# tgialoimtr/cnn_lstm_ctc_ocr

Measured on AMD Instinct MI355X. Metric: line-crops/sec (train step) at 32x256 bs=256; CER vs ref, higher is better.
Workload: dtype bf16

## Files before the change

### cnn_lstm_ctc_ocr_amd/_lib.py

```python
import ctypes
import os

import torch

_HERE = os.path.dirname(os.path.abspath(__file__))
LIB_PATH = os.environ.get("OCRK_LIB") or os.path.join(_HERE, "libocrk.so")

OCRK_OK = 0
OCRK_ERR_INVALID_ARG = 1
OCRK_ERR_HIP = 2
OCRK_ERR_INFEASIBLE = 3

F32 = 0
BF16 = 1

_p = ctypes.c_void_p
_i32 = ctypes.c_int
_u32 = ctypes.c_uint
_i64 = ctypes.c_int64
_f32 = ctypes.c_float
_sz = ctypes.c_size_t

SIGNATURES = {
    "ocrk_version": [],
# ... 70 lines not shown
    "ocrk_bn_relu_pool_bwd_slab": [_p, _p, _i32, _i32, _i32, _i32, _p, _p, _p, _p, _i32, _i32, _i32, _i32,
                                   _i32, _p, _p, _p, _i32, _p, _p, _sz, _i32, _p],
    "ocrk_lstm_fwd_step": [_p, _p, _p, _p, _p, _p, _i32, _i32, _i32, _i32, _p, _p, _p, _p, _i32, _p],
    "ocrk_lstm_bwd_step": [_p, _p, _p, _p, _p, _i32, _i32, _i32, _i32, _p, _p, _p, _p, _i32, _p],
    "ocrk_copy_batch": [_p, _i32, _i64, _p],
    "ocrk_gru_fwd_persistent_supported": [_i32, _i32],
    "ocrk_gru_fwd_persistent_workspace_size": [_i32, _i32],
    "ocrk_gru_fwd_persistent": [_p, _p, _p, _p, _i32, _i32, _i32, _p, _p, _p, _p, _p, _p, _p, _sz, _p],
    "ocrk_gru_bwd_persistent_supported": [_i32, _i32],
    "ocrk_gru_bwd_persistent_workspace_size": [_i32, _i32],
    "ocrk_gru_bwd_persistent": [_p, _p, _p, _i32, _i32, _i32, _p, _p, _p, _p, _p, _p, _p, _p, _sz, _p],
    "ocrk_persistent_flags_size": [_i32, _i32],
    "ocrk_lstm_fwd_persistent_supported": [_i32, _i32],
    "ocrk_lstm_fwd_persistent_workspace_size": [_i32, _i32],
    "ocrk_lstm_fwd_persistent": [_p, _p, _p, _i32, _i32, _i32, _p, _p, _p, _p, _p, _p, _p, _sz, _p],
    "ocrk_lstm_fwd_persistent_f32_supported": [_i32, _i32],
    "ocrk_lstm_fwd_persistent_f32_workspace_size": [_i32, _i32],
    "ocrk_lstm_fwd_persistent_f32_flags_size": [_i32, _i32],
    "ocrk_lstm_fwd_persistent_f32": [_p, _p, _p, _i32, _i32, _i32, _p, _p, _p, _p, _p, _p, _p, _sz, _p],
    "ocrk_lstm_bwd_persistent_f32_supported": [_i32, _i32],
    "ocrk_lstm_bwd_persistent_f32_workspace_size": [_i32, _i32],
    "ocrk_lstm_bwd_persistent_f32": [_p, _p, _i32, _i32, _i32, _p, _p, _p, _p, _p, _p, _p, _p, _sz, _p],
    "ocrk_lstm_bwd_persistent_supported": [_i32, _i32],
    "ocrk_lstm_bwd_persistent_workspace_size": [_i32, _i32],
    "ocrk_lstm_bwd_persistent_slices": [_i32, _i32],
    "ocrk_lstm_bwd_persistent": [_p, _p, _i32, _i32, _i32, _p, _p, _p, _p, _p, _p, _p, _p, _sz, _p],
    "ocrk_lstm_fwd": [_p, _p, _p, _p, _p, _i32, _i32, _i32, _p, _p, _p, _p, _i32, _p],
    "ocrk_lstm_bwd": [_p, _p, _p, _p, _i32, _i32, _i32, _p, _p, _p, _p, _i32, _p],
    "ocrk_gemm_workspace_size": [_i32, _i32, _i32, _i32],
    "ocrk_gemm": [_i32, _i32, _i32, _i32, _i32, _f32, _p, _i64, _i64, _p, _i64, _i64, _p, _i64, _i64,
                  _i32, _p, _i32, _i32, _i32, _i32, _i32, _p, _sz, _p],
    "ocrk_adam": [_p, _p, _p, _p, _i64, _f32, _f32, _f32, _f32, _f32, _p],
    "ocrk_adam_ex": [_p, _p, _p, _p, _i64, _f32, _f32, _f32, _f32, _f32, _u32, _p],
    "ocrk_cast": [_p, _i32, _p, _i32, _i64, _p],
    "ocrk_split_bf16": [_p, _i64, _p, _p, _p],
    "ocrk_permute3": [_p, _i32, _i32, _i32, _i32, _p, _i32, _p],
    "ocrk_strided_copy": [_p, _i64, _i64, _i64, _i64, _p, _i32, _i64, _i64, _p],
    "ocrk_colsum_workspace_size": [_i64, _i32],
    "ocrk_colsum": [_p, _i64, _i32, _i32, _p, _i32, _p, _sz, _p],
    "ocrk_slab_sum_workspace_size": [_i32],
    "ocrk_slab_sum": [_p, _i32, _i32, _i32, _p, _i32, _p, _sz, _p],
    "ocrk_relu_mask": [_p, _p, _i64, _f32, _p, _i32, _p],
    "ocrk_mul_scalar": [_p, _i64, _p, _p],
    "ocrk_mean": [_p, _i32, _p, _p],
    "ocrk_seq_len": [_p, _i32, _p, _p],
    "ocrk_timer_create": [_p],
    "ocrk_timer_record": [_p, _p],
    "ocrk_timer_elapsed": [_p, _p, _p],
    "ocrk_timer_destroy": [_p],
}
_RESTYPE = {"ocrk_last_error": ctypes.c_char_p}
_RESTYPE.update({n: ctypes.c_size_t for n in SIGNATURES if n.endswith("_workspace_size")})
_RESTYPE["ocrk_conv_stats_tiles"] = ctypes.c_size_t
_RESTYPE["ocrk_persistent_flags_size"] = ctypes.c_size_t
_RESTYPE["ocrk_bn_bwd_bias_slab_rows"] = ctypes.c_size_t
_RESTYPE["ocrk_bn_bwd_pooled_bias_slab_rows"] = ctypes.c_size_t
_RESTYPE["ocrk_crc32c"] = ctypes.c_uint32


class OcrkError(RuntimeError):

    def __init__(self, status, message):
        super().__init__(message)
        self.status = status


# ... 127 lines not shown
```

### cnn_lstm_ctc_ocr_amd/csrc/adam.hip

```cpp
#include "common.h"

template <bool ZERO>
__global__ void __launch_bounds__(256)
adam_kernel(float* __restrict__ p, float* __restrict__ g, float* __restrict__ m, float* __restrict__ v,
            int64_t n, float lr_t, float b1, float b2, float eps, float grad_scale) {
    const int64_t n4 = n / 4;
    const float c1 = 1.f - b1, c2 = 1.f - b2;
    for (int64_t i = (int64_t)blockIdx.x * 256 + threadIdx.x; i < n4; i += (int64_t)gridDim.x * 256) {
        float4 pp = reinterpret_cast<float4*>(p)[i], gg = reinterpret_cast<const float4*>(g)[i];
        float4 mm = reinterpret_cast<float4*>(m)[i], vv = reinterpret_cast<float4*>(v)[i];
        float* pe = &pp.x; float* ge = &gg.x; float* me = &mm.x; float* ve = &vv.x;
#pragma unroll
        for (int k = 0; k < 4; ++k) {
            float gk = ge[k] * grad_scale;
            me[k] += (gk - me[k]) * c1;
            ve[k] += (gk * gk - ve[k]) * c2;
            pe[k] -= lr_t * me[k] / (sqrtf(ve[k]) + eps);
        }
        reinterpret_cast<float4*>(p)[i] = pp;
        reinterpret_cast<float4*>(m)[i] = mm;
        reinterpret_cast<float4*>(v)[i] = vv;
        if constexpr (ZERO) reinterpret_cast<float4*>(g)[i] = make_float4(0.f, 0.f, 0.f, 0.f);
    }
    for (int64_t i = n4 * 4 + (int64_t)blockIdx.x * 256 + threadIdx.x; i < n; i += (int64_t)gridDim.x * 256) {
        float gk = g[i] * grad_scale;
        m[i] += (gk - m[i]) * c1;
        v[i] += (gk * gk - v[i]) * c2;
        p[i] -= lr_t * m[i] / (sqrtf(v[i]) + eps);
        if constexpr (ZERO) g[i] = 0.f;
    }
}

extern "C" int ocrk_adam_ex(float* p, float* g, float* m, float* v, int64_t n, float lr_t, float beta1,
                            float beta2, float eps, float grad_scale, unsigned flags, void* stream) {
    if (n == 0) return OCRK_OK;
    OCRK_REQUIRE(((uintptr_t)p | (uintptr_t)g | (uintptr_t)m | (uintptr_t)v) % 16 == 0, "ocrk_adam: buffers must be 16-B aligned");
    OCRK_REQUIRE((flags & ~(unsigned)OCRK_ADAM_ZERO_GRAD) == 0, "ocrk_adam_ex: unknown flags 0x%x", flags);
    unsigned grid = (unsigned)std::max<int64_t>(1, std::min<int64_t>(ocrk::cdiv(n / 4 + 1, 256), 4096));
    hipStream_t s = ocrk::as_stream(stream);
    if (flags & OCRK_ADAM_ZERO_GRAD)
        adam_kernel<true><<<grid, 256, 0, s>>>(p, g, m, v, n, lr_t, beta1, beta2, eps, grad_scale);
    else
        adam_kernel<false><<<grid, 256, 0, s>>>(p, g, m, v, n, lr_t, beta1, beta2, eps, grad_scale);
    return ocrk::launch_status("ocrk_adam");
}

extern "C" int ocrk_adam(float* p, const float* g, float* m, float* v, int64_t n, float lr_t, float beta1,
                         float beta2, float eps, float grad_scale, void* stream) {
    return ocrk_adam_ex(p, const_cast<float*>(g), m, v, n, lr_t, beta1, beta2, eps, grad_scale, 0u, stream);
}
```

### cnn_lstm_ctc_ocr_amd/kernels.py

```python
import ctypes

import torch

from . import _lib, options
from ._lib import ptr, call

F32, BF16 = _lib.F32, _lib.BF16
_DT = {torch.float32: F32, torch.bfloat16: BF16}


def dtype_code(dt):
    try:
        return _DT[dt]
    except KeyError:
        raise TypeError(f"unsupported dtype {dt}; libocrk computes in float32 or bfloat16")


def _stream(t):
    return _lib.stream_ptr(t.device)


def _chk(*ts):
    for t in ts:
        if t is None:
# ... 722 lines not shown
def colsum(x, M, N, out, accumulate=True):
    _chk(x, out)
    nb = _lib.lib().ocrk_colsum_workspace_size(M, N)
    ws = _ws(nb, x.device)
    call("ocrk_colsum", ptr(x), M, N, dtype_code(x.dtype), ptr(out), int(accumulate), ptr(ws), nb, _stream(x))


def relu_mask(dy, y, out_dtype, scale=1.0):
    _chk(dy, y)
    out = torch.empty(dy.shape, dtype=out_dtype, device=dy.device)
    call("ocrk_relu_mask", ptr(dy), ptr(y), dy.numel(), float(scale), ptr(out), dtype_code(out_dtype), _stream(dy))
    return out


def mul_scalar_(x, s):
    _chk(x, s)
    call("ocrk_mul_scalar", ptr(x), x.numel(), ptr(s), _stream(x))
    return x


def mean(x):
    _chk(x)
    out = torch.empty((), dtype=torch.float32, device=x.device)
    call("ocrk_mean", ptr(x), x.numel(), ptr(out), _stream(x))
    return out


def adam_(p, g, m, v, lr_t, beta1=0.9, beta2=0.999, eps=1e-8, grad_scale=1.0, zero_grad=False):
    _chk(p, g, m, v)
    call("ocrk_adam_ex", ptr(p), ptr(g), ptr(m), ptr(v), p.numel(), float(lr_t), float(beta1), float(beta2),
         float(eps), float(grad_scale), 1 if zero_grad else 0, _stream(p))


def ctc_loss(logits, labels, label_len, seq_len, grad_scale=1.0, need_grad=True, status=None):
    if logits.dtype != torch.float32:
        raise TypeError("ctc_loss takes float32 logits")
    _chk(logits, labels, label_len, seq_len)
    T, B, C = logits.shape
    Lmax = labels.shape[1] if labels.dim() == 2 else 0
    labels = labels.reshape(B, Lmax)
    if labels.numel() == 0:
        labels = torch.zeros(B, 1, dtype=torch.int32, device=logits.device)
        Lmax = 1
    nb = _lib.lib().ocrk_ctc_workspace_size(T, B, Lmax)
    ws = _ws(nb, logits.device)
    loss = torch.empty(B, dtype=torch.float32, device=logits.device)
    grad = torch.empty_like(logits) if need_grad else None
    if status is None:
        status = torch.empty(B, dtype=torch.int32, device=logits.device)
    call("ocrk_ctc_loss", ptr(logits), ptr(labels), ptr(label_len), ptr(seq_len), T, B, C, Lmax,
         float(grad_scale), ptr(loss), ptr(grad), ptr(status), ptr(status_word(logits.device)), ptr(ws), nb,
         _stream(logits))
    return loss, grad, status


def ctc_align(logits, labels, label_len, seq_len, status=None):
    if logits.dtype != torch.float32:
        raise TypeError("ctc_align takes float32 logits")
    _chk(logits, labels, label_len, seq_len)
    T, B, C = logits.shape
    Lmax = Lout = labels.shape[1] if labels.dim() == 2 else 0
    labels = labels.reshape(B, Lmax)
    if labels.numel() == 0:
        labels = torch.zeros(B, 1, dtype=torch.int32, device=logits.device)
        Lmax = 1
    nb = _lib.lib().ocrk_ctc_align_workspace_size(T, B, Lmax)
# ... 105 lines not shown
```

### cnn_lstm_ctc_ocr_amd/options.py

```python
import contextlib
import os

_HOST_DEFAULTS = {
    "LSTM_PERSISTENT": 1,
    "F32_TRAIN_EXACT": 0,
    "SIDE_STREAM": 1,
    "CONV_SIDE": 1,
    "CONV12_FUSED": 1,
    "RELU_BITS": 1,
    "POOLED_BN": 1,
    "CONV1_FUSED": 1,
    "CONV12_BWD": 1,
    "TN_ITEMS": 256,
    "TN_ITEMS_L1": 160,
}
KERNEL_OPTIONS = ("CONV_DIRECT", "CONV_ROWS", "CONV_ROWS_WIDE", "CONV_WGRAD_BLOCKS", "LSTM_SPIN_LIMIT",
                  "PERSIST_LATE", "LSTM_BWD_R16", "CTC_LDS",
                  "PP_PERSIST_NK", "NT_F32_EXACT", "NT_F32_MASK",
                  "NT_F32_X6", "BEAM_WAVE", "BN_BWD_BLOCKS", "BN_ROUTE", "BN_ROUTE_SEG", "BN_ROUTE_NCH", "CONV_TN_ITEMS", "CONV_TN4_ITEMS",
                  "CONV_WGRAD_CUS", "F32_MFMA", "GEMM_NT", "GEMM_NT_STAGED", "GEMM_PP", "GEMM_PPTN", "PP_MIN_N", "GEMM_TN",
                  "LSTM_DMA", "LSTM_BWD_DMA", "LSTM_FWD_R16", "NT_TAP_UNIFORM")


def _env_int(name, default):
    v = os.environ.get("OCRK_" + name)
    if v is None or v == "":
        return default
    try:
        return int(v)
    except ValueError:
        raise ValueError(f"OCRK_{name}={v!r}: an integer is expected") from None


_HOST = {k: _env_int(k, d) for k, d in _HOST_DEFAULTS.items()}


def get(name):
    if name in _HOST:
        return _HOST[name]
    if name in KERNEL_OPTIONS:
        import ctypes

        from . import _lib
        v = ctypes.c_int64()
        _lib.call("ocrk_get_option", name.encode(), ctypes.byref(v))
# ... 30 lines not shown
```

### cnn_lstm_ctc_ocr_amd/params.py

```python

import numpy as np
import torch

from . import kernels as K
from .config import LAYER_PARAMS, ModelConfig

_ALIGN = 64


def param_shapes(cfg):
    out = []
    cin = 1
    for filters, k, _pad, name, bn in LAYER_PARAMS:
        out.append((f"convnet/{name}/kernel", (k, k, cin, filters), True))
        out.append((f"convnet/{name}/bias", (filters,), True))
        if bn:
            out.append((f"convnet/{name}/batch_norm/gamma", (filters,), True))
            out.append((f"convnet/{name}/batch_norm/beta", (filters,), True))
            out.append((f"convnet/{name}/batch_norm/moving_mean", (filters,), False))
            out.append((f"convnet/{name}/batch_norm/moving_variance", (filters,), False))
        cin = filters
    n_in = cin
    for li, H in enumerate(cfg.rnn_sizes, start=1):
        pre = f"rnn/bdrnn{li}"
# ... 31 lines not shown
    return out[:i] + rnn + out[i:]


def _trunc_normal(rng, shape, std):
    x = rng.standard_normal(shape)
    bad = np.abs(x) > 2
    while bad.any():
        x[bad] = rng.standard_normal(int(bad.sum()))
        bad = np.abs(x) > 2
    return x * std


def reference_init(cfg, seed=0):
    rng = np.random.default_rng(seed)
    vals = {}
    shapes = {n: sh for n, sh, _t in param_shapes(cfg)}
    for name in creation_order(cfg):
        shape = shapes[name]
        leaf = name.rsplit("/", 1)[1]
        if name.startswith("convnet") and leaf == "kernel":
            v = _trunc_normal(rng, shape, np.sqrt(2.6 / (shape[0] * shape[1] * shape[2])))
        elif name == "rnn/logits/kernel":
            v = _trunc_normal(rng, shape, np.sqrt(2.6 / shape[0]))
        elif "gru_cell" in name or ("lstm_cell" in name and leaf == "kernel"):
            v = _trunc_normal(rng, shape, 0.01)
        elif leaf in ("gamma", "moving_variance"):
            v = np.ones(shape)
        else:
            v = np.zeros(shape)
        vals[name] = v.astype(np.float32)
    return vals


class ParamStore:
    def __init__(self, cfg=None, device="cuda", seed=0, values=None):
        self.cfg = cfg or ModelConfig()
        self.device = torch.device(device)
        self.spec = param_shapes(self.cfg)
        self.offsets = {}
        sizes = {True: 0, False: 0}
        for name, shape, tr in self.spec:
            n = int(np.prod(shape))
            self.offsets[name] = (tr, sizes[tr], shape)
            sizes[tr] += (n + _ALIGN - 1) // _ALIGN * _ALIGN
        self.n_trainable = sum(int(np.prod(s)) for _, s, tr in self.spec if tr)
        self.flat = torch.zeros(sizes[True], dtype=torch.float32, device=self.device)
        self.flat_grad = torch.zeros_like(self.flat)
        self.flat_stats = torch.zeros(max(sizes[False], _ALIGN), dtype=torch.float32, device=self.device)
        self.params, self.grads, self.stats = {}, {}, {}
        for name, shape, tr in self.spec:
            _, off, _ = self.offsets[name]
            n = int(np.prod(shape))
            if tr:
                self.params[name] = self.flat[off:off + n].view(shape)
                self.grads[name] = self.flat_grad[off:off + n].view(shape)
            else:
                self.stats[name] = self.flat_stats[off:off + n].view(shape)
        self.version = 0
        self._images = {}
        self.pending = []
        self.conv_late = []
        self.bn_group = None
        self.f32_conv_exact = False
        self.load_state_dict(values if values is not None else reference_init(self.cfg, seed))

    def state_dict(self):
# ... 39 lines not shown
        self._plan_fresh = False

    def images(self, key, builder):
        plan = self._plan_for(key)
        if plan is not None:
            if not self._plan_fresh:
                K.copy_batch(plan["table"], plan["njobs"], plan["tiles"], self.flat)
                self._plan_fresh = True
            return plan["images"][key]
        img = self._images.get(key)
        if img is None:
            img = builder()
            self._images[key] = img
        return img

    def _plan_for(self, key):
        if self.device.type != "cuda":
            return None
        dtype = key[-1]
        if dtype != self.cfg.dtype:
            return None
        plan = getattr(self, "_plan", None)
        if plan is None:
            plan = self._plan = self._build_plan(dtype)
            self._plan_fresh = False
        return plan if key in plan["images"] else None

    def _build_plan(self, dtype):
        dev = self.device
        esz = torch.empty(0, dtype=dtype).element_size()
        code = K.dtype_code(dtype)
        jobs, images = [], {}

        def job(src, s_off, rows, cols, in_rs, dst, d_off, out_rs, transpose):
            jobs.append([src.data_ptr() + 4 * s_off, dst.data_ptr() + esz * d_off, rows, cols, in_rs, out_rs, 0,
                         int(transpose) | (code << 32)])

        for li in range(2, 9):
            w = self.params[f"convnet/conv{li}/kernel"]
            kh, kw, cin, cout = w.shape
            w_nk = torch.empty(cout, kh * kw * cin, dtype=dtype, device=dev)
            w_bwd = torch.empty(cin, kh * kw * cout, dtype=dtype, device=dev)
            job(w, 0, kh * kw * cin, cout, cout, w_nk, 0, kh * kw * cin, True)
            for t in range(kh * kw):
                job(w, t * cin * cout, cin, cout, cout, w_bwd, t * cout, kh * kw * cout, False)
            images[("conv", f"conv{li}", dtype)] = (w_nk, w_bwd)
        for layer in range(1, len(self.cfg.rnn_sizes) + 1):
            pre = f"rnn/bdrnn{layer}"
            if self.cfg.cell == "lstm":
                kf = self.params[f"{pre}/fw/lstm_cell/kernel"]
                rows, G = kf.shape
                H = G // 4
                n_in = rows - H
                wxT = torch.empty(2 * G, n_in, dtype=dtype, device=dev)
                wx = torch.empty(n_in, 2 * G, dtype=dtype, device=dev)
                whT = torch.empty(2, G, H, dtype=dtype, device=dev)
                wh = torch.empty(2, H, G, dtype=dtype, device=dev)
                for d, dn in enumerate(("fw", "bw")):
                    k = self.params[f"{pre}/{dn}/lstm_cell/kernel"]
                    job(k, 0, n_in, G, G, wxT, d * G * n_in, n_in, True)
                    job(k, 0, n_in, G, G, wx, d * G, 2 * G, False)
                    job(k, n_in * G, H, G, G, whT, d * G * H, H, True)
                    job(k, n_in * G, H, G, G, wh, d * H * G, G, False)
                images[("lstm", layer, dtype)] = (wxT, wx, whT, wh, self.flat_bias_pair(layer))
            else:
                gk = self.params[f"{pre}/fw/gru_cell/gates/kernel"]
                rows, G2 = gk.shape
                H = G2 // 2
                n_in = rows - H
                G3 = 3 * H
                wxT = torch.empty(2 * G3, n_in, dtype=dtype, device=dev)
                wx = torch.empty(n_in, 2 * G3, dtype=dtype, device=dev)
                whgT = torch.empty(2, G2, H, dtype=dtype, device=dev)
                whcT = torch.empty(2, H, H, dtype=dtype, device=dev)
                whg = torch.empty(2, H, G2, dtype=dtype, device=dev)
                whc = torch.empty(2, H, H, dtype=dtype, device=dev)
                for d, dn in enumerate(("fw", "bw")):
                    g = self.params[f"{pre}/{dn}/gru_cell/gates/kernel"]
                    c = self.params[f"{pre}/{dn}/gru_cell/candidate/kernel"]
                    job(g, 0, n_in, G2, G2, wxT, d * G3 * n_in, n_in, True)
                    job(c, 0, n_in, H, H, wxT, (d * G3 + G2) * n_in, n_in, True)
                    job(g, 0, n_in, G2, G2, wx, d * G3, 2 * G3, False)
                    job(c, 0, n_in, H, H, wx, d * G3 + G2, 2 * G3, False)
                    job(g, n_in * G2, H, G2, G2, whgT, d * G2 * H, H, True)
                    job(c, n_in * H, H, H, H, whcT, d * H * H, H, True)
                    job(g, n_in * G2, H, G2, G2, whg, d * H * G2, G2, False)
                    job(c, n_in * H, H, H, H, whc, d * H * H, H, False)
                images[("gru", layer, dtype)] = (wxT, wx, whgT, whcT, whg, whc, self.gru_bias_cat(layer))
        lk = self.params["rnn/logits/kernel"]
        limg = torch.empty(lk.shape, dtype=dtype, device=dev)
        limgT = torch.empty(lk.shape[1], lk.shape[0], dtype=dtype, device=dev)
        job(lk, 0, lk.shape[0], lk.shape[1], lk.shape[1], limg, 0, lk.shape[1], False)
        job(lk, 0, lk.shape[0], lk.shape[1], lk.shape[1], limgT, 0, lk.shape[0], True)
        images[("logits", dtype)] = limg
        images[("logitsT", dtype)] = limgT
        tiles = 0
        for j in jobs:
            j[6] = tiles
            tiles += -(-j[2] // 32) * -(-j[3] // 32)
        table = torch.tensor(jobs, dtype=torch.int64).to(dev)
        return {"table": table, "njobs": len(jobs), "tiles": tiles, "images": images}

    def conv_images(self, name, dtype):
        def build():
            w = self.params[f"convnet/{name}/kernel"]
            kh, kw, cin, cout = w.shape
            w_nk = K.permute3(w, kh * kw * cin, cout, 1, dtype).view(cout, kh * kw * cin)
            w_bwd = K.permute3(w, kh * kw, cin, cout, dtype).view(cin, kh * kw * cout)
            return w_nk, w_bwd
        return self.images(("conv", name, dtype), build)

    def lstm_images(self, layer, dtype):
        def build():
            pre = f"rnn/bdrnn{layer}"
            kf = self.params[f"{pre}/fw/lstm_cell/kernel"]
            rows, G = kf.shape
            H = G // 4
            n_in = rows - H
            dev = kf.device
            wxT = torch.empty(2 * G, n_in, dtype=dtype, device=dev)
            wx = torch.empty(n_in, 2 * G, dtype=dtype, device=dev)
            whT = torch.empty(2, G, H, dtype=dtype, device=dev)
            wh = torch.empty(2, H, G, dtype=dtype, device=dev)
            for d, dn in enumerate(("fw", "bw")):
                k = self.params[f"{pre}/{dn}/lstm_cell/kernel"]
                K.strided_copy(k, n_in, G, G, 1, wxT, 1, n_in, out_offset=d * G * n_in)
                K.strided_copy(k, n_in, G, G, 1, wx, 2 * G, 1, out_offset=d * G)
                K.strided_copy(k, H, G, G, 1, whT, 1, H, out_offset=d * G * H, in_offset=n_in * G)
                K.strided_copy(k, H, G, G, 1, wh, G, 1, out_offset=d * H * G, in_offset=n_in * G)
            bias = self.flat_bias_pair(layer)
            return wxT, wx, whT, wh, bias
        return self.images(("lstm", layer, dtype), build)

    def flat_bias_pair(self, layer):
# ... 73 lines not shown
```

### cnn_lstm_ctc_ocr_amd/train.py

```python
import collections
import math
import time

import torch
import torch.distributed as dist

from . import _lib
from . import kernels as K
from . import options
from . import model as _model
from .config import TRAIN
from .model import check_feasible_host, convnet_layers, ctc_loss_layer, dense_labels, host_labels, rnn_layers




class GradBuckets:

    def __init__(self, store, group=None, comm=None, force=False):
        self.store, self.group, self.comm, self.force = store, group, comm, bool(force)
        rnn = [off for name, (tr, off, _s) in store.offsets.items() if tr and name.startswith("rnn/")]
        self.split = min(rnn) if rnn else store.flat_grad.numel()
        self.work = None
        self._stream = None
# ... 79 lines not shown
        dist.all_reduce(flat_grad, op=dist.ReduceOp.SUM, group=group)
    return 1.0 / world


class Trainer:

    def __init__(self, store, learning_rate=1e-4, momentum=0.9, decay_rate=0.9, decay_steps=2 ** 16,
                 decay_staircase=False, beta2=0.999, epsilon=1e-8, process_group=None, global_step=0,
                 summary=None, summary_every=100, sync_bn=False, comm=None, force_exchange=False):
        self.store = store
        self.sync_bn = bool(sync_bn)
        self.summary = summary
        self.summary_every = max(1, int(summary_every))
        self._summary_mark = None
        self.base_lr = learning_rate
        self.beta1 = momentum
        self.beta2 = beta2
        self.eps = epsilon
        self.decay_rate = decay_rate
        self.decay_steps = decay_steps
        self.staircase = decay_staircase
        self.group = process_group
        self.global_step = global_step
        self.m = torch.zeros_like(store.flat)
        self.v = torch.zeros_like(store.flat)
        self._grads_zeroed = False
        self._status_host = None
        self._status_ev = None
        self._status_stream = None
        self._status_ring = collections.deque()
        self.status_lag = 2
        self.buckets = GradBuckets(store, process_group, comm=comm, force=force_exchange)
        self.overlap_allreduce = True

    def learning_rate(self, step=None):
        step = self.global_step if step is None else step
        e = step / self.decay_steps
        if self.staircase:
            e = math.floor(e)
        return self.base_lr * self.decay_rate ** e

    def _bn_group(self):
        if not self.sync_bn or not (dist.is_available() and dist.is_initialized()):
            return None
        return self.group if self.group is not None else dist.group.WORLD

    def world_size(self):
        if self.buckets.comm is not None:
            return self.buckets.world()
        if dist.is_available() and dist.is_initialized():
            return dist.get_world_size(self.group)
        return 1

    def loss_and_grads(self, image, width, label):
        store = self.store
        if store.cfg.dtype != torch.float32:
            return self._loss_and_grads(image, width, label)
        if options.get("F32_TRAIN_EXACT"):
            with K.f32_exact():
                return self._loss_and_grads(image, width, label)
        prev, store.f32_conv_exact = store.f32_conv_exact, True
        try:
            return self._loss_and_grads(image, width, label)
        finally:
            store.f32_conv_exact = prev

    def _loss_and_grads(self, image, width, label):
        store = self.store
        prev_group, store.bn_group = store.bn_group, self._bn_group()
        try:
            return self._forward_backward(image, width, label)
        finally:
            store.bn_group = prev_group

    def _forward_backward(self, image, width, label):
        store = self.store
        if host_labels(label) and not (isinstance(width, torch.Tensor) and width.is_cuda):
            check_feasible_host(label, width)
        if self._grads_zeroed and not (store.device.type == "cuda" and torch.cuda.is_current_stream_capturing()):
            store.join()
        else:
            store.zero_grad()
        self._grads_zeroed = False
        features, seq_len = convnet_layers(image, width, TRAIN, store)
        if self.overlap_allreduce and features.requires_grad and self.buckets.active() and \
                not (features.is_cuda and torch.cuda.is_current_stream_capturing()):
            features.register_hook(self.buckets.rnn_ready)
        logits = rnn_layers(features, seq_len, store.cfg.num_classes, store)
        loss = ctc_loss_layer(logits, label, seq_len)
        if loss.dtype == torch.float32:
            _model.unit_backward(loss)
        else:
            loss.backward()
        return loss

    def reduce_gradients(self):
        self.store.join()
        return self.buckets.finish()

    def apply_gradients(self):
        store = self.store
        grad_scale = self.reduce_gradients()
        t = self.global_step + 1
        lr = self.learning_rate()
        lr_t = lr * math.sqrt(1 - self.beta2 ** t) / (1 - self.beta1 ** t)
        zero = store.device.type == "cuda"
        K.adam_(store.flat, store.flat_grad, self.m, self.v, lr_t, self.beta1, self.beta2, self.eps,
                grad_scale=grad_scale, zero_grad=zero)
        self._grads_zeroed = zero
        store.bump()
        self.global_step += 1

    def step(self, image, width, label):
        self.poll_status()
        lr = self.learning_rate()
        loss = self.loss_and_grads(image, width, label)
        self.apply_gradients()
        self.post_status()
        self.summarize(loss, lr, int(image.shape[0]))
        return loss

    def summarize(self, loss, lr, batch):
        if self.summary is None:
            return
        if self._summary_mark is not None and self.global_step % self.summary_every:
            return
        dev = self.store.device
        if dev.type == "cuda":
            now = torch.cuda.Event(enable_timing=True)
            now.record(torch.cuda.current_stream(dev))
        else:
            now = time.perf_counter()
        if self._summary_mark is None:
            self._summary_mark = (self.global_step, now)
        if self.global_step % self.summary_every:
            return
        s0, t0 = self._summary_mark
        crops = (self.global_step - s0) * batch * self.world_size()
        vals = {"learning_rate": lr, "loss": loss}
        if self.global_step > s0:
            if dev.type == "cuda":
                vals["crops_per_sec"] = lambda: round(crops / max(t0.elapsed_time(now) / 1e3, 1e-9), 2)
            elif now > t0:
                vals["crops_per_sec"] = round(crops / (now - t0), 2)
        self.summary.scalars(self.global_step, **vals)
        self._summary_mark = (self.global_step, now)

    def post_status(self):
        dev = self.store.device
# ... 110 lines not shown
```

### include/ocrk.h

```cpp
#ifndef OCRK_H_
#define OCRK_H_

#include <stddef.h>
#include <stdint.h>

#ifdef __cplusplus
extern "C" {
#endif

#define OCRK_ABI_VERSION 7

enum ocrk_status {
    OCRK_OK = 0,
    OCRK_ERR_INVALID_ARG = 1,
    OCRK_ERR_HIP = 2,
    OCRK_ERR_INFEASIBLE = 3
};

enum ocrk_dtype { OCRK_F32 = 0, OCRK_BF16 = 1 };

int ocrk_set_f32_gemm_mode(int mode);
int ocrk_f32_gemm_exact(void);

enum ocrk_device_status {
// ... 184 lines not shown
                 const int* seq_len, int T, int B, int H, const void* dout, const void* hprev_t,
                 const void* acts_t, void* dG_t, int dtype, void* stream);
int ocrk_gru_fwd_persistent_supported(int B, int H);
size_t ocrk_gru_fwd_persistent_workspace_size(int B, int H);
int ocrk_gru_fwd_persistent(const void* gx, const void* whgT, const void* whcT, const int* seq_len, int T, int B,
                            int H, void* out, void* hprev_t, void* rh_t, void* acts_t, unsigned* err,
                            unsigned* flags, void* ws, size_t ws_bytes, void* stream);
int ocrk_gru_bwd_persistent_supported(int B, int H);
size_t ocrk_gru_bwd_persistent_workspace_size(int B, int H);
int ocrk_gru_bwd_persistent(const void* whg, const void* whc, const int* seq_len, int T, int B, int H,
                            const void* dout, const void* hprev_t, const void* acts_t, void* dG_t, unsigned* err,
                            unsigned* flags, float* dbias_part, void* ws, size_t ws_bytes, void* stream);
size_t ocrk_persistent_flags_size(int B, int H);
int ocrk_lstm_fwd(const void* gx, const void* whT, void* h_state, float* c_state, const int* seq_len,
                  int T, int B, int H, void* out, void* hprev_t, float* cprev_t, void* acts_t, int dtype,
                  void* stream);
int ocrk_lstm_bwd(const void* wh, void* dg_state, float* dc_state, const int* seq_len, int T, int B, int H,
                  const void* dout, const float* cprev_t, const void* acts_t, void* dG_t, int dtype,
                  void* stream);

size_t ocrk_gemm_workspace_size(int M, int N, int batch, int splits);
int ocrk_gemm(int trans_a, int trans_b, int M, int N, int K, float alpha, const void* A, int64_t lda,
              int64_t stride_a, const void* B, int64_t ldb, int64_t stride_b, void* C, int64_t ldc,
              int64_t stride_c, int c_dtype, const float* bias, int relu, int accumulate, int batch,
              int dtype, int splits, void* ws, size_t ws_bytes, void* stream);

int ocrk_adam(float* p, const float* g, float* m, float* v, int64_t n, float lr_t, float beta1,
              float beta2, float eps, float grad_scale, void* stream);
#define OCRK_ADAM_ZERO_GRAD 1u
int ocrk_adam_ex(float* p, float* g, float* m, float* v, int64_t n, float lr_t, float beta1,
                 float beta2, float eps, float grad_scale, unsigned flags, void* stream);

int ocrk_copy_batch(const void* jobs, int njobs, int64_t total_tiles, void* stream);
int ocrk_cast(const void* in, int in_dtype, void* out, int out_dtype, int64_t n, void* stream);
int ocrk_permute3(const void* in, int in_dtype, int d0, int d1, int d2, void* out, int out_dtype,
                  void* stream);
int ocrk_strided_copy(const float* in, int64_t rows, int64_t cols, int64_t in_rs, int64_t in_cs, void* out,
                      int out_dtype, int64_t out_rs, int64_t out_cs, void* stream);
size_t ocrk_colsum_workspace_size(int64_t M, int N);
int ocrk_colsum(const void* in, int64_t M, int N, int dtype, float* out, int accumulate, void* ws,
                size_t ws_bytes, void* stream);
size_t ocrk_slab_sum_workspace_size(int nc);
int ocrk_slab_sum(const float* slab, int nslab, int nc, int ld, float* out, int accumulate, void* ws,
                  size_t ws_bytes, void* stream);
int ocrk_relu_mask(const float* dy, const float* y, int64_t n, float scale, void* out, int out_dtype,
                   void* stream);
int ocrk_mul_scalar(float* x, int64_t n, const float* s, void* stream);
int ocrk_mean(const float* x, int n, float* out, void* stream);
int ocrk_seq_len(const int* widths, int n, int* out, void* stream);

int ocrk_timer_create(void** ev);
int ocrk_timer_record(void* ev, void* stream);
int ocrk_timer_elapsed(void* ev0, void* ev1, float* ms);
int ocrk_timer_destroy(void* ev);

uint32_t ocrk_crc32c(const void* data, size_t n, uint32_t crc);

#ifdef __cplusplus
}
#endif
#endif
```

Before: 54110.

## Fuse Adam update with bf16/transposed weight-image refresh in one kernel

Adds an adam_images kernel that applies Adam to the flat fp32 parameters and, in the same pass, writes the updated values into the per-layer compute images (bf16 or f32, optionally transposed through a shared-memory tile). Contiguous gaps between image regions get ordinary vectorized Adam from a fixed set of workgroups. The goal is to drop the separate copy/cast pass that rebuilds weight images after every step, and to avoid re-reading parameters. It also adds an optional early-update path, off by default, that updates the tail of the parameters on a side stream during backward. The cost is a more complex region plan, and Adam's arithmetic now uses explicit FMAs, which can change rounding slightly.

Result: no change. 54220, median of 4 (+0.2%).

```diff
diff --git a/cnn_lstm_ctc_ocr_amd/_lib.py b/cnn_lstm_ctc_ocr_amd/_lib.py
--- a/cnn_lstm_ctc_ocr_amd/_lib.py
+++ b/cnn_lstm_ctc_ocr_amd/_lib.py
@@ -126,6 +126,8 @@
                   _i32, _p, _i32, _i32, _i32, _i32, _i32, _p, _sz, _p],
     "ocrk_adam": [_p, _p, _p, _p, _i64, _f32, _f32, _f32, _f32, _f32, _p],
     "ocrk_adam_ex": [_p, _p, _p, _p, _i64, _f32, _f32, _f32, _f32, _f32, _u32, _p],
+    "ocrk_adam_images_supported": [_i32],
+    "ocrk_adam_images": [_p, _p, _p, _p, _i64, _i64, _p, _i32, _i64, _i32, _f32, _f32, _f32, _f32, _f32, _u32, _p],
     "ocrk_cast": [_p, _i32, _p, _i32, _i64, _p],
     "ocrk_split_bf16": [_p, _i64, _p, _p, _p],
     "ocrk_permute3": [_p, _i32, _i32, _i32, _i32, _p, _i32, _p],
diff --git a/cnn_lstm_ctc_ocr_amd/csrc/adam.hip b/cnn_lstm_ctc_ocr_amd/csrc/adam.hip
--- a/cnn_lstm_ctc_ocr_amd/csrc/adam.hip
+++ b/cnn_lstm_ctc_ocr_amd/csrc/adam.hip
@@ -1,32 +1,27 @@
 #include "common.h"
+#include "adam_math.h"
 
 template <bool ZERO>
 __global__ void __launch_bounds__(256)
 adam_kernel(float* __restrict__ p, float* __restrict__ g, float* __restrict__ m, float* __restrict__ v,
             int64_t n, float lr_t, float b1, float b2, float eps, float grad_scale) {
     const int64_t n4 = n / 4;
-    const float c1 = 1.f - b1, c2 = 1.f - b2;
+    const AdamK a{lr_t, 1.f - b1, 1.f - b2, eps, grad_scale};
     for (int64_t i = (int64_t)blockIdx.x * 256 + threadIdx.x; i < n4; i += (int64_t)gridDim.x * 256) {
         float4 pp = reinterpret_cast<float4*>(p)[i], gg = reinterpret_cast<const float4*>(g)[i];
         float4 mm = reinterpret_cast<float4*>(m)[i], vv = reinterpret_cast<float4*>(v)[i];
         float* pe = &pp.x; float* ge = &gg.x; float* me = &mm.x; float* ve = &vv.x;
 #pragma unroll
-        for (int k = 0; k < 4; ++k) {
-            float gk = ge[k] * grad_scale;
-            me[k] += (gk - me[k]) * c1;
-            ve[k] += (gk * gk - ve[k]) * c2;
-            pe[k] -= lr_t * me[k] / (sqrtf(ve[k]) + eps);
-        }
+        for (int k = 0; k < 4; ++k) adam_update(pe[k], ge[k], me[k], ve[k], a);
         reinterpret_cast<float4*>(p)[i] = pp;
         reinterpret_cast<float4*>(m)[i] = mm;
         reinterpret_cast<float4*>(v)[i] = vv;
         if constexpr (ZERO) reinterpret_cast<float4*>(g)[i] = make_float4(0.f, 0.f, 0.f, 0.f);
     }
     for (int64_t i = n4 * 4 + (int64_t)blockIdx.x * 256 + threadIdx.x; i < n; i += (int64_t)gridDim.x * 256) {
-        float gk = g[i] * grad_scale;
-        m[i] += (gk - m[i]) * c1;
-        v[i] += (gk * gk - v[i]) * c2;
-        p[i] -= lr_t * m[i] / (sqrtf(v[i]) + eps);
+        float pi = p[i], mi = m[i], vi = v[i];
+        adam_update(pi, g[i], mi, vi, a);
+        p[i] = pi; m[i] = mi; v[i] = vi;
         if constexpr (ZERO) g[i] = 0.f;
     }
 }
diff --git a/cnn_lstm_ctc_ocr_amd/csrc/adam_images.hip b/cnn_lstm_ctc_ocr_amd/csrc/adam_images.hip
--- /dev/null
+++ b/cnn_lstm_ctc_ocr_amd/csrc/adam_images.hip
@@ -0,0 +1,227 @@
+#include "common.h"
+#include "adam_math.h"
+
+namespace {
+
+struct AdamDst {
+    void* p;
+    int64_t rs;
+    int64_t transpose;
+};
+struct AdamRegion {
+    int64_t begin, rows, cols, tile0, ndst;
+    AdamDst d[2];
+    int64_t reserved;
+};
+static_assert(sizeof(AdamRegion) == 12 * 8, "region layout (include/ocrk.h)");
+
+constexpr int TR = 64, TC = 64;
+constexpr int MAX_REGIONS = 512;
+constexpr int GAP_WGS = 256;
+
+__device__ __forceinline__ void adam4(float4& pp, const float4& gg, float4& mm, float4& vv, const AdamK& a) {
+    float* pe = &pp.x; const float* ge = &gg.x; float* me = &mm.x; float* ve = &vv.x;
+#pragma unroll
+    for (int k = 0; k < 4; ++k) adam_update(pe[k], ge[k], me[k], ve[k], a);
+}
+
+template <bool BF>
+__device__ __forceinline__ void store4(void* dst, int64_t off, float o0, float o1, float o2, float o3) {
+    if constexpr (BF) {
+        typedef unsigned int u32x2_t __attribute__((ext_vector_type(2)));
+        u32x2_t w;
+        w[0] = (unsigned)__builtin_bit_cast(unsigned short, (bf16)o0) |
+               ((unsigned)__builtin_bit_cast(unsigned short, (bf16)o1) << 16);
+        w[1] = (unsigned)__builtin_bit_cast(unsigned short, (bf16)o2) |
+               ((unsigned)__builtin_bit_cast(unsigned short, (bf16)o3) << 16);
+        *reinterpret_cast<u32x2_t*>(reinterpret_cast<bf16*>(dst) + off) = w;
+    } else {
+        *reinterpret_cast<float4*>(reinterpret_cast<float*>(dst) + off) = make_float4(o0, o1, o2, o3);
+    }
+}
+
+template <bool BF>
+__device__ __forceinline__ void store1(void* dst, int64_t off, float x) {
+    if constexpr (BF) reinterpret_cast<bf16*>(dst)[off] = (bf16)x;
+    else reinterpret_cast<float*>(dst)[off] = x;
+}
+
+template <bool ZERO>
+__device__ __forceinline__ void update1(float* p, float* g, float* m, float* v, int64_t i, const AdamK& a) {
+    float pp = p[i], mm = m[i], vv = v[i];
+    adam_update(pp, g[i], mm, vv, a);
+    p[i] = pp; m[i] = mm; v[i] = vv;
+    if constexpr (ZERO) g[i] = 0.f;
+}
+
+template <bool ZERO, bool BF>
+__global__ void __launch_bounds__(256)
+adam_images_kernel(float* __restrict__ p, float* __restrict__ g, float* __restrict__ m, float* __restrict__ v,
+                   int64_t begin, int64_t end, const AdamRegion* __restrict__ regions, int nregions,
+                   int total_tiles, float lr_t, float b1, float b2, float eps, float grad_scale) {
+    __shared__ float tile[TR][TC + 1];
+    __shared__ int first[MAX_REGIONS];
+    const AdamK a{lr_t, 1.f - b1, 1.f - b2, eps, grad_scale};
+    const int tid = threadIdx.x;
+
+    if ((int)blockIdx.x < GAP_WGS) {
+        const int ngaps = nregions + 1;
+        const int groups = min(ngaps, GAP_WGS), per = GAP_WGS / groups;
+        const int group = blockIdx.x % groups, lane = blockIdx.x / groups;
+        if (lane >= per) return;
+        for (int i = group; i < ngaps; i += groups) {
+            int64_t lo = begin, hi = end;
+            if (i > 0) lo = max(lo, regions[i - 1].begin + regions[i - 1].rows * regions[i - 1].cols);
+            if (i < nregions) hi = min(hi, regions[i].begin);
+            if (lo >= hi) continue;
+            const int64_t lo4 = min(hi, (lo + 3) & ~(int64_t)3), hi4 = max(lo4, hi & ~(int64_t)3);
+            for (int64_t i4 = lo4 / 4 + (int64_t)lane * 256 + tid; i4 < hi4 / 4; i4 += (int64_t)per * 256) {
+                float4 pp = reinterpret_cast<float4*>(p)[i4], gg = reinterpret_cast<const float4*>(g)[i4];
+                float4 mm = reinterpret_cast<float4*>(m)[i4], vv = reinterpret_cast<float4*>(v)[i4];
+                adam4(pp, gg, mm, vv, a);
+                reinterpret_cast<float4*>(p)[i4] = pp;
+                reinterpret_cast<float4*>(m)[i4] = mm;
+                reinterpret_cast<float4*>(v)[i4] = vv;
+                if constexpr (ZERO) reinterpret_cast<float4*>(g)[i4] = make_float4(0.f, 0.f, 0.f, 0.f);
+            }
+            if (lane == 0) {
+                if (lo + tid < lo4) update1<ZERO>(p, g, m, v, lo + tid, a);
+                if (hi4 + tid < hi) update1<ZERO>(p, g, m, v, hi4 + tid, a);
+            }
+        }
+        return;
+    }
+
+    for (int i = tid; i < nregions; i += 256) first[i] = (int)regions[i].tile0;
+    __syncthreads();
+    const int t = blockIdx.x - GAP_WGS;
+    if (t >= total_tiles) return;
+    int lo = 0, hi = nregions - 1;
+    while (lo < hi) {
+        const int mid = (lo + hi + 1) >> 1;
+        if (first[mid] <= t) lo = mid; else hi = mid - 1;
+    }
+    const AdamRegion R = regions[lo];
+    const int64_t lt = t - R.tile0, tc = (R.cols + TC - 1) / TC;
+    const int64_t r0 = (lt / tc) * TR, c0 = (lt % tc) * TC;
+    const int ndst = (int)R.ndst;
+    bool any_t = false, vec = ((R.begin | R.rows | R.cols) & 3) == 0;
+#pragma unroll
+    for (int d = 0; d < 2; ++d) {
+        if (d >= ndst) continue;
+        any_t |= R.d[d].transpose != 0;
+        vec &= (R.d[d].rs & 3) == 0 && ((uintptr_t)R.d[d].p & (BF ? 7 : 15)) == 0;
+    }
+    if (R.begin < begin || R.begin + R.rows * R.cols > end) return;
+
+    if (vec) {
+        const int q = tid >> 4, c4 = (tid & 15) * 4;
+        const int64_t c = c0 + c4;
+        float4 pp[4], gg[4], mm[4], vv[4];
+        bool ok[4];
+#pragma unroll
+        for (int k = 0; k < 4; ++k) {
+            const int64_t r = r0 + q + 16 * k;
+            ok[k] = r < R.rows && c < R.cols;
+            if (ok[k]) {
+                const int64_t i4 = (R.begin + r * R.cols + c) / 4;
+                pp[k] = reinterpret_cast<float4*>(p)[i4]; gg[k] = reinterpret_cast<const float4*>(g)[i4];
+                mm[k] = reinterpret_cast<float4*>(m)[i4]; vv[k] = reinterpret_cast<float4*>(v)[i4];
+            }
+        }
+#pragma unroll
+        for (int k = 0; k < 4; ++k) {
+            if (!ok[k]) continue;
+            const int64_t r = r0 + q + 16 * k;
+            const int64_t i4 = (R.begin + r * R.cols + c) / 4;
+            adam4(pp[k], gg[k], mm[k], vv[k], a);
+            reinterpret_cast<float4*>(p)[i4] = pp[k];
+            reinterpret_cast<float4*>(m)[i4] = mm[k];
+            reinterpret_cast<float4*>(v)[i4] = vv[k];
+            if constexpr (ZERO) reinterpret_cast<float4*>(g)[i4] = make_float4(0.f, 0.f, 0.f, 0.f);
+#pragma unroll
+            for (int d = 0; d < 2; ++d)
+                if (d < ndst && !R.d[d].transpose) store4<BF>(R.d[d].p, r * R.d[d].rs + c, pp[k].x, pp[k].y, pp[k].z, pp[k].w);
+            if (any_t) {
+                float* row = &tile[q + 16 * k][c4];
+                row[0] = pp[k].x; row[1] = pp[k].y; row[2] = pp[k].z; row[3] = pp[k].w;
+            }
+        }
+        if (!any_t) return;
+        __syncthreads();
+#pragma unroll
+        for (int d = 0; d < 2; ++d) {
+            if (d >= ndst || !R.d[d].transpose) continue;
+#pragma unroll
+            for (int k = 0; k < 4; ++k) {
+                const int oc = q + 16 * k;
+                const int64_t orow = c0 + oc, ocol = r0 + c4;
+                if (orow >= R.cols || ocol >= R.rows) continue;
+                store4<BF>(R.d[d].p, orow * R.d[d].rs + ocol, tile[c4][oc], tile[c4 + 1][oc], tile[c4 + 2][oc],
+                           tile[c4 + 3][oc]);
+            }
+        }
+        return;
+    }
+
+    for (int i = tid; i < TR * TC; i += 256) {
+        const int rr = i / TC, cc = i % TC;
+        const int64_t r = r0 + rr, c = c0 + cc;
+        if (r >= R.rows || c >= R.cols) continue;
+        const int64_t idx = R.begin + r * R.cols + c;
+        float pv = p[idx], mv = m[idx], vvv = v[idx];
+        adam_update(pv, g[idx], mv, vvv, a);
+        p[idx] = pv; m[idx] = mv; v[idx] = vvv;
+        if constexpr (ZERO) g[idx] = 0.f;
+#pragma unroll
+        for (int d = 0; d < 2; ++d)
+            if (d < ndst && !R.d[d].transpose) store1<BF>(R.d[d].p, r * R.d[d].rs + c, pv);
+        if (any_t) tile[rr][cc] = pv;
+    }
+    if (!any_t) return;
+    __syncthreads();
+#pragma unroll
+    for (int d = 0; d < 2; ++d) {
+        if (d >= ndst || !R.d[d].transpose) continue;
+        for (int i = tid; i < TR * TC; i += 256) {
+            const int oc = i / TR, rr = i % TR;
+            if (c0 + oc >= R.cols || r0 + rr >= R.rows) continue;
+            store1<BF>(R.d[d].p, (c0 + oc) * R.d[d].rs + r0 + rr, tile[rr][oc]);
+        }
+    }
+}
+
+}
+
+extern "C" int ocrk_adam_images_supported(int image_dtype) {
+    return image_dtype == OCRK_F32 || image_dtype == OCRK_BF16;
+}
+
+extern "C" int ocrk_adam_images(float* p, float* g, float* m, float* v, int64_t begin, int64_t end,
+                                const void* regions, int nregions, int64_t total_tiles, int image_dtype, float lr_t,
+                                float beta1, float beta2, float eps, float grad_scale, unsigned flags, void* stream) {
+    OCRK_REQUIRE(ocrk_adam_images_supported(image_dtype), "ocrk_adam_images: image dtype=%d not covered", image_dtype);
+    OCRK_REQUIRE(begin >= 0 && begin <= end, "ocrk_adam_images: bad range [%lld, %lld)", (long long)begin,
+                 (long long)end);
+    OCRK_REQUIRE(nregions >= 0 && nregions <= MAX_REGIONS && (nregions == 0 || regions != nullptr),
+                 "ocrk_adam_images: nregions=%d out of range (0..%d)", nregions, MAX_REGIONS);
+    OCRK_REQUIRE(total_tiles >= 0 && total_tiles < (1ll << 30) && (nregions > 0 || total_tiles == 0),
+                 "ocrk_adam_images: nregions=%d tiles=%lld", nregions, (long long)total_tiles);
+    OCRK_REQUIRE(((uintptr_t)p | (uintptr_t)g | (uintptr_t)m | (uintptr_t)v) % 16 == 0,
+                 "ocrk_adam_images: buffers must be 16-B aligned");
+    OCRK_REQUIRE((flags & ~(unsigned)OCRK_ADAM_ZERO_GRAD) == 0, "ocrk_adam_images: unknown flags 0x%x", flags);
+    if (begin == end) return OCRK_OK;
+    const unsigned grid = (unsigned)total_tiles + GAP_WGS;
+    const AdamRegion* R = (const AdamRegion*)regions;
+    hipStream_t s = ocrk::as_stream(stream);
+    const bool zero = flags & OCRK_ADAM_ZERO_GRAD, bf = image_dtype == OCRK_BF16;
+#define OCRK_AI_LAUNCH(Z, B)                                                                                     \
+    adam_images_kernel<Z, B><<<grid, 256, 0, s>>>(p, g, m, v, begin, end, R, nregions, (int)total_tiles, lr_t, \
+                                                   beta1, beta2, eps, grad_scale)
+    if (zero && bf) OCRK_AI_LAUNCH(true, true);
+    else if (zero) OCRK_AI_LAUNCH(true, false);
+    else if (bf) OCRK_AI_LAUNCH(false, true);
+    else OCRK_AI_LAUNCH(false, false);
+#undef OCRK_AI_LAUNCH
+    return ocrk::launch_status("ocrk_adam_images");
+}
diff --git a/cnn_lstm_ctc_ocr_amd/csrc/adam_math.h b/cnn_lstm_ctc_ocr_amd/csrc/adam_math.h
--- /dev/null
+++ b/cnn_lstm_ctc_ocr_amd/csrc/adam_math.h
@@ -0,0 +1,13 @@
+#pragma once
+
+struct AdamK {
+    float lr_t, c1, c2, eps, grad_scale;
+};
+
+__device__ __forceinline__ void adam_update(float& p, float g, float& m, float& v, const AdamK& a) {
+#pragma clang fp contract(off)
+    const float gk = g * a.grad_scale;
+    m = __builtin_fmaf(a.c1, __builtin_fmaf(g, a.grad_scale, -m), m);
+    v = __builtin_fmaf(a.c2, __builtin_fmaf(gk, gk, -v), v);
+    p = p - a.lr_t * m / (sqrtf(v) + a.eps);
+}
diff --git a/cnn_lstm_ctc_ocr_amd/kernels.py b/cnn_lstm_ctc_ocr_amd/kernels.py
--- a/cnn_lstm_ctc_ocr_amd/kernels.py
+++ b/cnn_lstm_ctc_ocr_amd/kernels.py
@@ -778,6 +778,19 @@
          float(eps), float(grad_scale), 1 if zero_grad else 0, _stream(p))
 
 
+def adam_images_supported(dtype):
+    code = _DT.get(dtype)
+    return code is not None and bool(_lib.lib().ocrk_adam_images_supported(code))
+
+
+def adam_images_(p, g, m, v, begin, end, table, nregions, total_tiles, image_dtype, lr_t, beta1=0.9, beta2=0.999,
+                 eps=1e-8, grad_scale=1.0, zero_grad=False):
+    _chk(p, g, m, v, table)
+    call("ocrk_adam_images", ptr(p), ptr(g), ptr(m), ptr(v), int(begin), int(end), ptr(table), int(nregions),
+         int(total_tiles), dtype_code(image_dtype), float(lr_t), float(beta1), float(beta2), float(eps),
+         float(grad_scale), 1 if zero_grad else 0, _stream(p))
+
+
 def ctc_loss(logits, labels, label_len, seq_len, grad_scale=1.0, need_grad=True, status=None):
     if logits.dtype != torch.float32:
         raise TypeError("ctc_loss takes float32 logits")
diff --git a/cnn_lstm_ctc_ocr_amd/options.py b/cnn_lstm_ctc_ocr_amd/options.py
--- a/cnn_lstm_ctc_ocr_amd/options.py
+++ b/cnn_lstm_ctc_ocr_amd/options.py
@@ -11,6 +11,8 @@
     "POOLED_BN": 1,
     "CONV1_FUSED": 1,
     "CONV12_BWD": 1,
+    "ADAM_IMAGES": 1,
+    "EARLY_UPDATE": 0,
     "TN_ITEMS": 256,
     "TN_ITEMS_L1": 160,
 }
diff --git a/cnn_lstm_ctc_ocr_amd/params.py b/cnn_lstm_ctc_ocr_amd/params.py
--- a/cnn_lstm_ctc_ocr_amd/params.py
+++ b/cnn_lstm_ctc_ocr_amd/params.py
@@ -87,6 +87,47 @@
     return vals
 
 
+REGION_TILE = 64
+REGION_WORDS = 12
+
+
+def plan_regions(jobs, esz):
+    cuts = set()
+    for s, rows, cols, in_rs, _d, _rs, _t in jobs:
+        if in_rs != cols or rows < 1 or cols < 1:
+            return None
+        cuts.update((s, s + rows * cols))
+    cuts = sorted(cuts)
+    regions = {}
+    for s, rows, cols, _in_rs, dst, out_rs, transpose in jobs:
+        inner = [c for c in cuts if s <= c <= s + rows * cols]
+        for a, b in zip(inner, inner[1:]):
+            if (a - s) % cols or (b - s) % cols:
+                return None
+            r0 = (a - s) // cols
+            reg = regions.setdefault(a, (a, (b - a) // cols, cols, []))
+            if reg[1:3] != ((b - a) // cols, cols) or len(reg[3]) == 2:
+                return None
+            reg[3].append((dst + esz * (r0 if transpose else r0 * out_rs), out_rs, int(bool(transpose))))
+    return [regions[a] for a in sorted(regions)]
+
+
+def region_records(regions, begin, end):
+    rows, tiles = [], 0
+    for a, nr, nc, dsts in regions:
+        b = a + nr * nc
+        if b <= begin or a >= end:
+            continue
+        if a < begin or b > end:
+            return None
+        rec = [a, nr, nc, tiles, len(dsts)]
+        for d in list(dsts) + [(0, 0, 0)] * (2 - len(dsts)):
+            rec += list(d)
+        rows.append(rec + [0])
+        tiles += -(-nr // REGION_TILE) * -(-nc // REGION_TILE)
+    return rows, tiles
+
+
 class ParamStore:
     def __init__(self, cfg=None, device="cuda", seed=0, values=None):
         self.cfg = cfg or ModelConfig()
@@ -192,9 +233,14 @@
         code = K.dtype_code(dtype)
         jobs, images = [], {}
 
+        flat_ptr = self.flat.data_ptr()
+        sources = []
+
         def job(src, s_off, rows, cols, in_rs, dst, d_off, out_rs, transpose):
             jobs.append([src.data_ptr() + 4 * s_off, dst.data_ptr() + esz * d_off, rows, cols, in_rs, out_rs, 0,
                          int(transpose) | (code << 32)])
+            sources.append(((src.data_ptr() - flat_ptr) // 4 + s_off, rows, cols, in_rs,
+                            dst.data_ptr() + esz * d_off, out_rs, bool(transpose)))
 
         for li in range(2, 9):
             w = self.params[f"convnet/conv{li}/kernel"]
@@ -259,7 +305,41 @@
             j[6] = tiles
             tiles += -(-j[2] // 32) * -(-j[3] // 32)
         table = torch.tensor(jobs, dtype=torch.int64).to(dev)
-        return {"table": table, "njobs": len(jobs), "tiles": tiles, "images": images}
+        return {"table": table, "njobs": len(jobs), "tiles": tiles, "images": images, "dtype": dtype,
+                "regions": plan_regions(sources, esz), "region_tables": {}}
+
+    def region_table(self, begin, end):
+        plan = getattr(self, "_plan", None)
+        if plan is None or plan["regions"] is None or not K.adam_images_supported(plan["dtype"]):
+            return None
+        key = (int(begin), int(end))
+        if key not in plan["region_tables"]:
+            rec = region_records(plan["regions"], *key)
+            if rec is not None:
+                rows, tiles = rec
+                t = torch.tensor(rows, dtype=torch.int64).reshape(len(rows), REGION_WORDS).to(self.device)
+                rec = (t, len(rows), tiles)
+            plan["region_tables"][key] = rec
+        return plan["region_tables"][key]
+
+    def fused_update(self, m, v, begin, end, lr_t, beta1, beta2, eps, grad_scale, zero_grad):
+        tab = self.region_table(begin, end)
+        if tab is None:
+            return False
+        table, n, tiles = tab
+        K.adam_images_(self.flat, self.flat_grad, m, v, begin, end, table, n, tiles, self._plan["dtype"], lr_t,
+                       beta1, beta2, eps, grad_scale=grad_scale, zero_grad=zero_grad)
+        return True
+
+    def images_current(self, ranges):
+        plan = getattr(self, "_plan", None)
+        if plan is None or not plan["regions"]:
+            return False
+        for a, nr, nc, _d in plan["regions"]:
+            if not any(b <= a and a + nr * nc <= e for b, e in ranges):
+                return False
+        self._plan_fresh = True
+        return True
 
     def conv_images(self, name, dtype):
         def build():
diff --git a/cnn_lstm_ctc_ocr_amd/train.py b/cnn_lstm_ctc_ocr_amd/train.py
--- a/cnn_lstm_ctc_ocr_amd/train.py
+++ b/cnn_lstm_ctc_ocr_amd/train.py
@@ -135,6 +135,10 @@
         self.status_lag = 2
         self.buckets = GradBuckets(store, process_group, comm=comm, force=force_exchange)
         self.overlap_allreduce = True
+        self._early_armed = False
+        self._early = None
+        self._early_stream = None
+        self._own_stream = None
 
     def learning_rate(self, step=None):
         step = self.global_step if step is None else step
@@ -180,6 +184,7 @@
         store = self.store
         if host_labels(label) and not (isinstance(width, torch.Tensor) and width.is_cuda):
             check_feasible_host(label, width)
+        self._drop_early()
         if self._grads_zeroed and not (store.device.type == "cuda" and torch.cuda.is_current_stream_capturing()):
             store.join()
         else:
@@ -189,6 +194,8 @@
         if self.overlap_allreduce and features.requires_grad and self.buckets.active() and \
                 not (features.is_cuda and torch.cuda.is_current_stream_capturing()):
             features.register_hook(self.buckets.rnn_ready)
+        if features.requires_grad and self._early_wanted():
+            features.register_hook(self._early_update)
         logits = rnn_layers(features, seq_len, store.cfg.num_classes, store)
         loss = ctc_loss_layer(logits, label, seq_len)
         if loss.dtype == torch.float32:
@@ -201,23 +208,80 @@
         self.store.join()
         return self.buckets.finish()
 
+    def _lr_t(self):
+        t = self.global_step + 1
+        return self.learning_rate() * math.sqrt(1 - self.beta2 ** t) / (1 - self.beta1 ** t)
+
+    def _early_wanted(self):
+        store = self.store
+        return (self._early_armed and store.device.type == "cuda" and options.get("ADAM_IMAGES")
+                and options.get("EARLY_UPDATE") and not self.buckets.active()
+                and not torch.cuda.is_current_stream_capturing()
+                and 0 < self.buckets.split < store.flat.numel())
+
+    def _early_update(self, *_):
+        store = self.store
+        split, n = self.buckets.split, store.flat.numel()
+        if self._early is not None or store.region_table(split, n) is None:
+            return
+        dev = store.device
+        es = _model._SIDE_STREAMS.get((dev, "side")) if options.get("EARLY_UPDATE") != 2 else None
+        if es is None:
+            if self._own_stream is None:
+                self._own_stream = torch.cuda.Stream(dev)
+            es = self._own_stream
+        self._early_stream = es
+        K.fork(es, torch.cuda.current_stream(dev))
+        for ev in store.pending:
+            K.wait_mark(es, ev)
+        with torch.cuda.stream(es):
+            store.fused_update(self.m, self.v, split, n, self._lr_t(), self.beta1, self.beta2, self.eps,
+                               grad_scale=1.0, zero_grad=True)
+            done = torch.cuda.Event()
+            done.record(es)
+        self._early = done
+
+    def _drop_early(self):
+        if self._early is not None:
+            K.wait_mark(torch.cuda.current_stream(self.store.device), self._early)
+            self._early = None
+            self.store.bump()
+
     def apply_gradients(self):
         store = self.store
         grad_scale = self.reduce_gradients()
-        t = self.global_step + 1
-        lr = self.learning_rate()
-        lr_t = lr * math.sqrt(1 - self.beta2 ** t) / (1 - self.beta1 ** t)
+        lr_t = self._lr_t()
         zero = store.device.type == "cuda"
-        K.adam_(store.flat, store.flat_grad, self.m, self.v, lr_t, self.beta1, self.beta2, self.eps,
-                grad_scale=grad_scale, zero_grad=zero)
+        n = store.flat.numel()
+        adam = dict(beta1=self.beta1, beta2=self.beta2, eps=self.eps, grad_scale=grad_scale, zero_grad=zero)
+        early, self._early = self._early, None
+        fused = []
+        if early is not None:
+            split = self.buckets.split
+            if store.fused_update(self.m, self.v, 0, split, lr_t, **adam):
+                fused.append((0, split))
+            else:
+                K.adam_(store.flat[:split], store.flat_grad[:split], self.m[:split], self.v[:split], lr_t, **adam)
+            K.wait_mark(torch.cuda.current_stream(store.device), early)
+            fused.append((split, n))
+        elif zero and options.get("ADAM_IMAGES") and store.fused_update(self.m, self.v, 0, n, lr_t, **adam):
+            fused.append((0, n))
+        else:
+            K.adam_(store.flat, store.flat_grad, self.m, self.v, lr_t, **adam)
         self._grads_zeroed = zero
         store.bump()
+        if fused:
+            store.images_current(fused)
         self.global_step += 1
 
     def step(self, image, width, label):
         self.poll_status()
         lr = self.learning_rate()
-        loss = self.loss_and_grads(image, width, label)
+        self._early_armed = True
+        try:
+            loss = self.loss_and_grads(image, width, label)
+        finally:
+            self._early_armed = False
         self.apply_gradients()
         self.post_status()
         self.summarize(loss, lr, int(image.shape[0]))
diff --git a/include/ocrk.h b/include/ocrk.h
--- a/include/ocrk.h
+++ b/include/ocrk.h
@@ -240,6 +240,10 @@
                  float beta2, float eps, float grad_scale, unsigned flags, void* stream);
 
 int ocrk_copy_batch(const void* jobs, int njobs, int64_t total_tiles, void* stream);
+int ocrk_adam_images_supported(int image_dtype);
+int ocrk_adam_images(float* p, float* g, float* m, float* v, int64_t begin, int64_t end, const void* regions,
+                     int nregions, int64_t total_tiles, int image_dtype, float lr_t, float beta1, float beta2,
+                     float eps, float grad_scale, unsigned flags, void* stream);
 int ocrk_cast(const void* in, int in_dtype, void* out, int out_dtype, int64_t n, void* stream);
 int ocrk_permute3(const void* in, int in_dtype, int d0, int d1, int d2, void* out, int out_dtype,
                   void* stream);
```
